# yassouali/pytorch-segmentation

Hardware: NVIDIA H100
Metric: images/sec DeepLabV3+/ResNet101 513x513 train step (fwd+CE+bwd+SGD) (higher is better)
Workload: dtype bf16

## Files before the change

### pytorch-segmentation_b200/csrc/seg_conv_tc.cu

```cuda
#include <cuda.h>
#include <mutex>
#include <stdlib.h>
#include "seg_common.cuh"
#include "seg_ptx.cuh"
#include "seg_sync.cuh"

namespace seg {
namespace tc {

using namespace ptx;

constexpr int BM = 128;
constexpr int BK = 64;
constexpr int A_BYTES = BM * 128;
constexpr int KIND_KK = 0, KIND_KM = 1;
constexpr int NTHREADS = 384;
constexpr int NCONS = 256;
constexpr int MAXT = 49;

constexpr int BAR_CONSUMERS = 1;
constexpr int BAR_ORDER = 2;
constexpr int BAR_WG = 4;

struct TcParams {
  CUtensorMap mapA;
  CUtensorMap mapB;
  int M;
  int Ncols;
  int taps;
  int kchunks;
  int stride;
  int lower_h, lower_w;
  int PQ, Q;
  int x_im2col;
  int brows_per_tap;
  short tap_wt[MAXT];
  short tap_oh[MAXT];
  short tap_ow[MAXT];
  void* out;
  long long ldo;
  int out_dtype;
  float beta;
  const float* bias;
  double* stats;
  int stat_rows;
  unsigned* stat_ticket;
  SyncDesc sync;
  int out_strided, out_H, out_W, osy, osx, opy, opx;
  int n_tiles, tiles;
  int kblocks_total, kblocks_per_split;
  float* dw;
  int dw_K, dw_C;
  float* ws;
};

__device__ __forceinline__ void row_to_coords(int m, int PQ, int Q, int stride, int lower_h, int lower_w, int& n, int& h,
                                              int& w) {
  n = m / PQ;
  int rem = m - n * PQ;
  int pp = rem / Q;
  int qq = rem - pp * Q;
  h = lower_h + pp * stride;
  w = lower_w + qq * stride;
}

template <int BN, int TA, int TB>
__device__ __forceinline__ void wgmma_tile(float* acc, uint64_t adesc, uint64_t bdesc, uint32_t accumulate) {
  if constexpr (BN == 64) wgmma_m64n64k16<TA, TB>(acc, adesc, bdesc, accumulate);
  else if constexpr (BN == 128) wgmma_m64n128k16<TA, TB>(acc, adesc, bdesc, accumulate);
  else wgmma_m64n256k16<TA, TB>(acc, adesc, bdesc, accumulate);
}

template <int BN, int KIND>
__device__ __forceinline__ void load_kblock(const TcParams& p, uint32_t a_dst, uint32_t bar, int kc, int wtap, uint16_t oh,
                                            uint16_t ow, int n_img, int h0, int w0, int m0, int n0) {
  const uint32_t b_dst = a_dst + A_BYTES;
  if (p.x_im2col)
    tma_load_im2col_4d(a_dst, &p.mapA, bar, kc * BK, w0, h0, n_img, ow, oh);
  else
    tma_load_2d(a_dst, &p.mapA, bar, kc * BK, m0);
  if (KIND == KIND_KK) {
    tma_load_2d(b_dst, &p.mapB, bar, kc * BK, wtap * p.brows_per_tap + n0);
  } else {
#pragma unroll
    for (int j = 0; j < BN / 64; ++j)
      tma_load_2d(b_dst + j * 8192, &p.mapB, bar, n0 + j * 64, wtap * p.brows_per_tap + kc * BK);
  }
}

template <int BN>
__device__ __forceinline__ void stage_acc(const float* acc, const float* acc1, uint8_t* stage, int rbase, int warp, int lane,
                                          const float* bias, bool out_f32) {
  const int esize = out_f32 ? 4 : 2;
  const int CPR = BN * esize / 16;
  const int swz = (CPR >= 32 ? 31 : CPR - 1);
  const int r0 = rbase + warp * 16 + (lane >> 2);
#pragma unroll
  for (int j = 0; j < BN / 8; ++j) {
    const int col = j * 8 + 2 * (lane & 3);
    float b0 = 0.f, b1 = 0.f;
    if (bias) {
      b0 = bias[col];
      b1 = bias[col + 1];
    }
#pragma unroll
    for (int h = 0; h < 4; ++h) {
      if (h >= 2 && !acc1) break;
      const float* a = h < 2 ? acc : acc1;
      const int r = r0 + 8 * (h & 1) + 32 * (h & 2);
      const float x0 = a[4 * j + 2 * (h & 1)] + b0, x1 = a[4 * j + 2 * (h & 1) + 1] + b1;
      const int byte = col * esize;
      uint8_t* dst = stage + (size_t)r * (BN * esize) + ((((byte >> 4) ^ (r & swz))) << 4) + (byte & 15);
      if (out_f32)
        *reinterpret_cast<float2*>(dst) = make_float2(x0, x1);
      else
        *reinterpret_cast<__nv_bfloat162*>(dst) = __floats2bfloat162_rn(x0, x1);
    }
  }
}


template <int BN, int ESIZE>
__device__ __forceinline__ void store_tile(const TcParams& p, const uint8_t* stage, int tid, int m0, int n0, int ncols_tile) {
  constexpr int CPR = BN * ESIZE / 16;
  constexpr int swz = (CPR >= 32 ? 31 : CPR - 1);
  constexpr int RSTEP = 128 / CPR;
  constexpr int NCH = BM / RSTEP;
  constexpr int BATCH = 8;
  static_assert(128 % CPR == 0 && NCH % BATCH == 0, "chunk walk of the staged tile");
  const int c16 = tid % CPR;
  const int nchunks = (ncols_tile * ESIZE + 15) >> 4;
  if (c16 >= nchunks) return;
  const bool vec_ok = ((p.ldo * ESIZE) & 15) == 0 && ((reinterpret_cast<uintptr_t>(p.out) + (size_t)n0 * ESIZE) & 15) == 0;
  const int first_col = (c16 << 4) / ESIZE;
  const bool full = first_col + 16 / ESIZE <= ncols_tile;
  auto row_dst = [&](int tr) {
    const int grow = m0 + tr;
    long long pixel = grow;
    if (p.out_strided) {
      const int n = grow / p.PQ;
      const int rem = grow - n * p.PQ;
      const int i = rem / p.Q, jj = rem - i * p.Q;
      pixel = ((long long)n * p.out_H + (i * p.osy + p.opy)) * p.out_W + (jj * p.osx + p.opx);
    }
    return reinterpret_cast<uint8_t*>(p.out) + ((size_t)pixel * p.ldo + n0) * ESIZE + ((size_t)c16 << 4);
  };
  auto row_src = [&](int tr) { return stage + (size_t)tr * (BN * ESIZE) + ((c16 ^ (tr & swz)) << 4); };
  if (ESIZE == 2 && vec_ok && full && p.beta != 0.f) {
    for (int b = 0; b < NCH; b += BATCH) {
      uint8_t* dst[BATCH];
      uint4 old[BATCH];
#pragma unroll
      for (int u = 0; u < BATCH; ++u) {
        const int tr = tid / CPR + (b + u) * RSTEP;
        dst[u] = m0 + tr < p.M ? row_dst(tr) : nullptr;
        old[u] = dst[u] ? *reinterpret_cast<const uint4*>(dst[u]) : make_uint4(0u, 0u, 0u, 0u);
      }
#pragma unroll
      for (int u = 0; u < BATCH; ++u) {
        if (!dst[u]) continue;
        float a[8], o[8];
        unpack8(*reinterpret_cast<const bf16x8*>(row_src(tid / CPR + (b + u) * RSTEP)), a);
        unpack8(*reinterpret_cast<const bf16x8*>(&old[u]), o);
#pragma unroll
        for (int k = 0; k < 8; ++k) a[k] += p.beta * o[k];
        *reinterpret_cast<bf16x8*>(dst[u]) = pack8(a);
      }
    }
    return;
  }
  for (int tr = tid / CPR; tr < BM; tr += RSTEP) {
    if (m0 + tr >= p.M) break;
    const uint8_t* src = row_src(tr);
    uint8_t* dst = row_dst(tr);
    if (ESIZE == 2 && vec_ok && full) {
      *reinterpret_cast<bf16x8*>(dst) = *reinterpret_cast<const bf16x8*>(src);
    } else if (ESIZE == 2) {
      float a[8];
      unpack8(*reinterpret_cast<const bf16x8*>(src), a);
      __nv_bfloat16* d = reinterpret_cast<__nv_bfloat16*>(dst);
      for (int k = 0; k < 8; ++k)
        if (first_col + k < ncols_tile) {
          float o = a[k];
          if (p.beta != 0.f) o += p.beta * bf2f(d[k]);
          d[k] = f2bf(o);
        }
    } else {
      const float4 val = *reinterpret_cast<const float4*>(src);
      const float a[4] = {val.x, val.y, val.z, val.w};
      float* d = reinterpret_cast<float*>(dst);
      if (vec_ok && full && p.beta == 0.f) {
        *reinterpret_cast<float4*>(d) = val;
      } else {
        for (int k = 0; k < 4; ++k)
          if (first_col + k < ncols_tile) d[k] = (p.beta != 0.f) ? a[k] + p.beta * d[k] : a[k];
      }
    }
  }
}

template <int BN>
struct PPCfg {
  static_assert(BN == 64 || BN == 128, "ping-pong tile width");
  static constexpr int B_BYTES = BN * 128;
  static constexpr int STAGE_BYTES = A_BYTES + B_BYTES;
  static constexpr int STAGES = BN == 64 ? 6 : 4;
  static constexpr int RING = STAGES * STAGE_BYTES;
  static constexpr int STG_BYTES = BM * 256;
  static constexpr int MAXG = BM / 32;
  static constexpr int STAT_BYTES = MAXG * 2 * BN * 4 + BN * 4;
  static constexpr int SMEM = RING + 2 * (STG_BYTES + STAT_BYTES) + 1024  + 256 ;
  static_assert(16 * STAGES + 8 <= 256, "barrier area");
  static_assert(SMEM <= 227 * 1024, "shared memory per block");
};

template <int BN, int KIND>
__global__ void __launch_bounds__(NTHREADS, 1) conv_gemm_pp(const __grid_constant__ TcParams p) {
  using C = PPCfg<BN>;
  constexpr int STAGES = C::STAGES;
  extern __shared__ uint8_t smem_raw[];
  const uint32_t raw_addr = smem_u32(smem_raw);
  const uint32_t smem0 = (raw_addr + 1023u) & ~1023u;
  uint8_t* smem_gen = smem_raw + (smem0 - raw_addr);
  const uint32_t bar0 = smem0 + C::RING + 2 * (C::STG_BYTES + C::STAT_BYTES);
  auto full_bar = [&](int s) { return bar0 + 8u * s; };
  auto empty_bar = [&](int s) { return bar0 + 8u * (STAGES + s); };
  volatile int* flag_sm = reinterpret_cast<volatile int*>(smem_gen + (bar0 - smem0) + 16 * STAGES);

  const int num_iters = p.taps * p.kchunks;
  const int grid = gridDim.x;
  const int ntiles = (p.tiles - (int)blockIdx.x + grid - 1) / grid;

  if (threadIdx.x == 0) {
    prefetch_tmap(&p.mapA);
    prefetch_tmap(&p.mapB);
    for (int s = 0; s < STAGES; ++s) {
      mbar_init(full_bar(s), 1);
      mbar_init(empty_bar(s), 4);
    }
    fence_mbar_init();
  }
  __syncthreads();
  pdl_wait();

  if (threadIdx.x < 128) {
    setmaxnreg_dec<40>();
    if (threadIdx.x == 0 && num_iters > 0) {
      int it = 0;
      for (int j = 0; j < ntiles; ++j) {
        const int t = blockIdx.x + j * grid;
        const int m0 = (t / p.n_tiles) * BM, n0 = (t % p.n_tiles) * BN;
        int n_img = 0, h0 = 0, w0 = 0;
        if (p.x_im2col) row_to_coords(m0, p.PQ, p.Q, p.stride, p.lower_h, p.lower_w, n_img, h0, w0);
        for (int tap = 0; tap < p.taps; ++tap) {
          const int wtap = p.tap_wt[tap];
          const uint16_t oh = (uint16_t)p.tap_oh[tap], ow = (uint16_t)p.tap_ow[tap];
          for (int kc = 0; kc < p.kchunks; ++kc, ++it) {
            const int st = it % STAGES;
            mbar_wait_nocall(empty_bar(st), ((it / STAGES) & 1) ^ 1u);
            mbar_arrive_expect_tx(full_bar(st), C::STAGE_BYTES);
            load_kblock<BN, KIND>(p, smem0 + st * C::STAGE_BYTES, full_bar(st), kc, wtap, oh, ow, n_img, h0, w0, m0, n0);
          }
        }
      }
    }
    return;
  }

  setmaxnreg_inc<232>();
  const int cw = (threadIdx.x - 128) >> 7;
  const int tid = threadIdx.x & 127;
  const int warp = tid >> 5, lane = tid & 31;
  uint8_t* stage = smem_gen + C::RING + cw * C::STG_BYTES;
  float* stat_sm = reinterpret_cast<float*>(smem_gen + C::RING + 2 * C::STG_BYTES + cw * C::STAT_BYTES);
  float* bias_sm = stat_sm + C::MAXG * 2 * BN;
  const bool out_f32 = p.out_dtype != SEG_DT_BF16;
  const int esize = out_f32 ? 4 : 2;
  const int CPR = BN * esize / 16;
  const int swz = (CPR >= 32 ? 31 : CPR - 1);
  auto wg_sync = [&] { named_sync(BAR_WG + cw, 128); };

  for (int j = cw; j < ntiles; j += 2) {
    const int t = blockIdx.x + j * grid;
    const int m0 = (t / p.n_tiles) * BM, n0 = (t % p.n_tiles) * BN;
    float acc0[BN / 2], acc1[BN / 2];
#pragma unroll
    for (int i = 0; i < BN / 2; ++i) acc0[i] = acc1[i] = 0.f;

    if (j > 0) named_sync(BAR_ORDER + cw, NCONS);
    {
      constexpr int TB = (KIND == KIND_KK) ? 0 : 1;
      const int it0 = j * num_iters;
      for (int i = 0; i < num_iters; ++i) {
        const int it = it0 + i;
        const int st = it % STAGES;
        mbar_wait_nocall(full_bar(st), (it / STAGES) & 1);
        const uint32_t a_addr = smem0 + st * C::STAGE_BYTES;
        const uint32_t b_addr = a_addr + A_BYTES;
        const uint64_t adesc0 = make_smem_desc_sw128(a_addr, 16, 1024);
        const uint64_t adesc1 = make_smem_desc_sw128(a_addr + 8192, 16, 1024);
        const uint64_t bdesc0 = make_smem_desc_sw128(b_addr, TB ? 8192 : 16, 1024);
        wgmma_fence();
#pragma unroll
        for (int k = 0; k < BK / 16; ++k) {
          const uint64_t bdesc = bdesc0 + (uint64_t)(TB ? (k * 2048 >> 4) : (k * 32 >> 4));
          wgmma_tile<BN, 0, TB>(acc0, adesc0 + (uint64_t)(k * 32 >> 4), bdesc, 1u);
          wgmma_tile<BN, 0, TB>(acc1, adesc1 + (uint64_t)(k * 32 >> 4), bdesc, 1u);
        }
        wgmma_commit();
        wgmma_wait<1>();
        __syncwarp();
        if (i > 0 && lane == 0) mbar_arrive(empty_bar((it - 1) % STAGES));
      }
      if (j + 1 < ntiles) named_arrive(BAR_ORDER + (cw ^ 1), NCONS);
      wgmma_wait<0>();
      __syncwarp();
      if (num_iters > 0 && lane == 0) mbar_arrive(empty_bar((it0 + num_iters - 1) % STAGES));
    }

    const int ncols_tile = min(BN, p.Ncols - n0);
    if (p.bias && tid < BN) bias_sm[tid] = tid < ncols_tile ? __ldg(p.bias + n0 + tid) : 0.f;
    wg_sync();
    stage_acc<BN>(acc0, acc1, stage, 0, warp, lane, p.bias ? bias_sm : nullptr, out_f32);
    wg_sync();

    const int ngroups = BM / p.stat_rows;
    if (p.stats) {
      const int parts = min(128 / BN, ngroups);
      const int rpp = BM / parts;
      const int c = tid % BN, part = tid / BN;
      const int rvalid = min(BM, p.M - m0);
      if (part < parts) {
        const int byte = c * esize;
        int g = part * rpp / p.stat_rows;
        auto load = [&](int r) {
          const uint8_t* src = stage + (size_t)r * (BN * esize) + ((((byte >> 4) ^ (r & swz))) << 4) + (byte & 15);
          return out_f32 ? *reinterpret_cast<const float*>(src) : bf2f(*reinterpret_cast<const __nv_bfloat16*>(src));
        };
        for (int rg = part * rpp; rg < (part + 1) * rpp; rg += p.stat_rows, ++g) {
          float s1 = 0.f, s2 = 0.f;
          const int rend = min(rg + p.stat_rows, rvalid);
          int r = rg;
          for (; r + 8 <= rend; r += 8) {
            float x[8];
#pragma unroll
            for (int u = 0; u < 8; ++u) x[u] = load(r + u);
#pragma unroll
            for (int u = 0; u < 8; ++u) {
              s1 += x[u];
              s2 = fmaf(x[u], x[u], s2);
            }
          }
          for (; r < rend; ++r) {
            const float x = load(r);
            s1 += x;
            s2 = fmaf(x, x, s2);
          }
          stat_sm[(g * 2 + 0) * BN + c] = s1;
          stat_sm[(g * 2 + 1) * BN + c] = s2;
        }
      }
    }

    if (out_f32)
      store_tile<BN, 4>(p, stage, tid, m0, n0, ncols_tile);
    else
      store_tile<BN, 2>(p, stage, tid, m0, n0, ncols_tile);
    if (j == ntiles - 1 && tid == 0) pdl_trigger();

    if (p.stats) {
      wg_sync();
      if (tid < ncols_tile) {
        float a = 0.f, b = 0.f;
        for (int g = 0; g < ngroups; ++g) {
          a += stat_sm[(g * 2 + 0) * BN + tid];
          b += stat_sm[(g * 2 + 1) * BN + tid];
        }
        atomicAdd(p.stats + n0 + tid, (double)a);
        atomicAdd(p.stats + p.Ncols + n0 + tid, (double)b);
      }
    }
  }

  if (p.stats && p.sync.world > 0)
    sync_push_when_last<false>(p.sync, p.stats, 2 * p.Ncols, p.stat_ticket, gridDim.x, threadIdx.x - 128, NCONS,
                               [] { named_sync(BAR_CONSUMERS, NCONS); }, flag_sm);
}


template <int BN>
struct Cfg {
  static constexpr int B_BYTES = BN * 128;
  static constexpr int STAGE_BYTES = A_BYTES + B_BYTES;
  static constexpr int STAGES = BN == 64 ? 6 : (BN == 128 ? 5 : 4);
  static constexpr int SMEM = STAGES * STAGE_BYTES + 1024  + 256 ;
  static_assert(STAGES * STAGE_BYTES >= BM * BN * 4, "staging tile must fit in the pipeline ring");
  static_assert(SMEM <= 227 * 1024, "shared memory per block");
};

template <int BN>
__global__ void __launch_bounds__(NTHREADS, 1) conv_gemm_wgrad(const __grid_constant__ TcParams p) {
  using C = Cfg<BN>;
  constexpr int STAGES = C::STAGES;
  extern __shared__ uint8_t smem_raw[];
  const uint32_t raw_addr = smem_u32(smem_raw);
  const uint32_t smem0 = (raw_addr + 1023u) & ~1023u;
  uint8_t* smem_gen = smem_raw + (smem0 - raw_addr);
  const uint32_t bar0 = smem0 + STAGES * C::STAGE_BYTES;
  auto full_bar = [&](int s) { return bar0 + 8u * s; };
  auto empty_bar = [&](int s) { return bar0 + 8u * (STAGES + s); };

  const int m0 = blockIdx.x * BM;
  const int n0 = blockIdx.y * BN;

  const int tap_mm = blockIdx.z % p.taps;
  const int split = blockIdx.z / p.taps;
  const int kb_begin = split * p.kblocks_per_split;
  const int kb_end = min(kb_begin + p.kblocks_per_split, p.kblocks_total);
  const int num_iters = max(kb_end - kb_begin, 0);

  if (threadIdx.x == 0) {
    prefetch_tmap(&p.mapA);
    prefetch_tmap(&p.mapB);
    for (int s = 0; s < STAGES; ++s) {
      mbar_init(full_bar(s), 1);
      mbar_init(empty_bar(s), 8);
    }
    fence_mbar_init();
  }
  __syncthreads();
  pdl_wait();

  if (threadIdx.x < 128) {
    if (threadIdx.x == 0 && num_iters > 0) {
      const uint16_t oh = (uint16_t)p.tap_oh[tap_mm], ow = (uint16_t)p.tap_ow[tap_mm];
      int it = 0;
      for (int kb = kb_begin; kb < kb_end; ++kb, ++it) {
        const int st = it % STAGES;
        const uint32_t ph = (it / STAGES) & 1;
        mbar_wait_nocall(empty_bar(st), ph ^ 1u);
        const uint32_t a_dst = smem0 + st * C::STAGE_BYTES;
        const uint32_t b_dst = a_dst + A_BYTES;
        const int pix0 = kb * BK;
        mbar_arrive_expect_tx(full_bar(st), C::STAGE_BYTES);
        tma_load_2d(a_dst, &p.mapA, full_bar(st), m0, pix0);
        tma_load_2d(a_dst + 8192, &p.mapA, full_bar(st), m0 + 64, pix0);
        if (p.x_im2col) {
          int n_img, h0, w0;
          row_to_coords(pix0, p.PQ, p.Q, p.stride, p.lower_h, p.lower_w, n_img, h0, w0);
#pragma unroll
          for (int j = 0; j < BN / 64; ++j)
            tma_load_im2col_4d(b_dst + j * 8192, &p.mapB, full_bar(st), n0 + j * 64, w0, h0, n_img, ow, oh);
        } else {
#pragma unroll
          for (int j = 0; j < BN / 64; ++j) tma_load_2d(b_dst + j * 8192, &p.mapB, full_bar(st), n0 + j * 64, pix0);
        }
      }
    }
    return;
  }

  if (num_iters == 0) return;
  const int ctid = threadIdx.x - 128;
  const int cw = ctid >> 7;
  const int warp = (ctid >> 5) & 3, lane = ctid & 31;
  float acc[BN / 2];
#pragma unroll
  for (int i = 0; i < BN / 2; ++i) acc[i] = 0.f;
  for (int it = 0; it < num_iters; ++it) {
    const int st = it % STAGES;
    mbar_wait_nocall(full_bar(st), (it / STAGES) & 1);
    const uint32_t a_addr = smem0 + st * C::STAGE_BYTES + cw * 8192;
    const uint32_t b_addr = smem0 + st * C::STAGE_BYTES + A_BYTES;
    const uint64_t adesc0 = make_smem_desc_sw128(a_addr, 8192, 1024);
    const uint64_t bdesc0 = make_smem_desc_sw128(b_addr, 8192, 1024);
    wgmma_fence();
#pragma unroll
    for (int k = 0; k < BK / 16; ++k)
      wgmma_tile<BN, 1, 1>(acc, adesc0 + (uint64_t)(k * 2048 >> 4), bdesc0 + (uint64_t)(k * 2048 >> 4), 1u);
    wgmma_commit();
    wgmma_wait<1>();
    __syncwarp();
    if (it > 0 && lane == 0) mbar_arrive(empty_bar((it - 1) % STAGES));
  }
  wgmma_wait<0>();
  named_sync(BAR_CONSUMERS, NCONS);

  uint8_t* stage = smem_gen;
  const int ncols_tile = min(BN, p.Ncols - n0);
  stage_acc<BN>(acc, nullptr, stage, cw * 64, warp, lane, nullptr, true);
  named_sync(BAR_CONSUMERS, NCONS);

  const int CPR = BN * 4 / 16;
  const int swz = (CPR >= 32 ? 31 : CPR - 1);
  float* base = p.ws ? p.ws + (size_t)split * p.taps * p.dw_K * p.dw_C : p.dw;
  for (int idx = ctid; idx < BM * CPR; idx += NCONS) {
    const int tr = idx / CPR, c16 = idx - tr * CPR;
    const int row = m0 + tr, col0 = c16 * 4;
    if (row >= p.M || col0 >= ncols_tile) continue;
    const float4 v = *reinterpret_cast<const float4*>(stage + (size_t)tr * (BN * 4) + ((c16 ^ (tr & swz)) << 4));
    float* dst = base + ((size_t)tap_mm * p.dw_K + row) * p.dw_C + n0 + col0;
    const bool vec = col0 + 4 <= ncols_tile && ((reinterpret_cast<uintptr_t>(dst) & 15) == 0);
    const float a[4] = {v.x, v.y, v.z, v.w};
    if (p.ws) {
      if (vec)
        *reinterpret_cast<float4*>(dst) = v;
      else
        for (int i = 0; i < 4; ++i)
          if (col0 + i < ncols_tile) dst[i] = a[i];
    } else if (vec) {
      asm volatile("red.global.add.v4.f32 [%0], {%1, %2, %3, %4};" ::"l"(dst), "f"(v.x), "f"(v.y), "f"(v.z), "f"(v.w)
                   : "memory");
    } else {
      for (int i = 0; i < 4; ++i)
        if (col0 + i < ncols_tile) atomicAdd(dst + i, a[i]);
    }
  }
}

typedef CUresult (*EncodeTiledFn)(CUtensorMap*, CUtensorMapDataType, cuuint32_t, void*, const cuuint64_t*,
                                  const cuuint64_t*, const cuuint32_t*, const cuuint32_t*, CUtensorMapInterleave,
                                  CUtensorMapSwizzle, CUtensorMapL2promotion, CUtensorMapFloatOOBfill);
typedef CUresult (*EncodeIm2colFn)(CUtensorMap*, CUtensorMapDataType, cuuint32_t, void*, const cuuint64_t*,
                                   const cuuint64_t*, const int*, const int*, cuuint32_t, cuuint32_t,
                                   const cuuint32_t*, CUtensorMapInterleave, CUtensorMapSwizzle,
                                   CUtensorMapL2promotion, CUtensorMapFloatOOBfill);
static EncodeTiledFn g_encode_tiled = nullptr;
static EncodeIm2colFn g_encode_im2col = nullptr;
static int g_driver_version = 0;

static int resolve_driver() {
  static std::once_flag once;
  static int status = 0;
  std::call_once(once, [] {
    void* f1 = nullptr;
    void* f2 = nullptr;
    cudaDriverEntryPointQueryResult q;
    if (cudaGetDriverEntryPoint("cuTensorMapEncodeTiled", &f1, cudaEnableDefault, &q) != cudaSuccess || !f1) status = 1;
    if (cudaGetDriverEntryPoint("cuTensorMapEncodeIm2col", &f2, cudaEnableDefault, &q) != cudaSuccess || !f2) status = 1;
    g_encode_tiled = (EncodeTiledFn)f1;
    g_encode_im2col = (EncodeIm2colFn)f2;
    cudaDriverGetVersion(&g_driver_version);
  });
  if (status) set_error("cannot resolve cuTensorMapEncode* driver entry points");
  return status;
}

static int make_map_2d(CUtensorMap* m, const void* ptr, int64_t rows, int64_t cols, int64_t ld, int box_rows) {
  if (resolve_driver()) return 1;
  SEG_REQUIRE((reinterpret_cast<uintptr_t>(ptr) & 15) == 0, "TMA: base pointer not 16-byte aligned");
  SEG_REQUIRE(ld % 8 == 0, "TMA: row pitch %lld not a multiple of 8 elements", (long long)ld);
  cuuint64_t dims[2] = {(cuuint64_t)cols, (cuuint64_t)rows};
  cuuint64_t strides[1] = {(cuuint64_t)ld * 2};
  cuuint32_t box[2] = {64, (cuuint32_t)box_rows};
  cuuint32_t es[2] = {1, 1};
  CUresult r = g_encode_tiled(m, CU_TENSOR_MAP_DATA_TYPE_BFLOAT16, 2, const_cast<void*>(ptr), dims, strides, box, es,
                              CU_TENSOR_MAP_INTERLEAVE_NONE, CU_TENSOR_MAP_SWIZZLE_128B,
                              CU_TENSOR_MAP_L2_PROMOTION_L2_256B, CU_TENSOR_MAP_FLOAT_OOB_FILL_NONE);
  SEG_REQUIRE(r == CUDA_SUCCESS, "cuTensorMapEncodeTiled failed (%d) rows=%lld cols=%lld ld=%lld box_rows=%d", (int)r,
              (long long)rows, (long long)cols, (long long)ld, box_rows);
  return 0;
}

static int make_map_im2col(CUtensorMap* m, const void* ptr, int N, int H, int W, int C, int64_t ld, int lower_w,
                           int lower_h, int upper_w, int upper_h, int stride, int pixels) {
  if (resolve_driver()) return 1;
  SEG_REQUIRE((reinterpret_cast<uintptr_t>(ptr) & 15) == 0, "TMA: base pointer not 16-byte aligned");
  SEG_REQUIRE(ld % 8 == 0, "TMA: channel pitch %lld not a multiple of 8", (long long)ld);
  SEG_REQUIRE(lower_w >= -128 && upper_w >= -128 && lower_w <= 127 && upper_w <= 127 && lower_h >= -128 &&
                  upper_h >= -128 && lower_h <= 127 && upper_h <= 127,
              "im2col corner out of range");
  cuuint64_t dims[4] = {(cuuint64_t)C, (cuuint64_t)W, (cuuint64_t)H, (cuuint64_t)N};
  cuuint64_t strides[3] = {(cuuint64_t)ld * 2, (cuuint64_t)W * ld * 2, (cuuint64_t)H * W * ld * 2};
  int lo[2] = {lower_w, lower_h};
  int up[2] = {upper_w, upper_h};
  cuuint32_t es[4] = {1, (cuuint32_t)stride, (cuuint32_t)stride, 1};
  CUresult r = g_encode_im2col(m, CU_TENSOR_MAP_DATA_TYPE_BFLOAT16, 4, const_cast<void*>(ptr), dims, strides, lo, up,
                               64, (cuuint32_t)pixels, es, CU_TENSOR_MAP_INTERLEAVE_NONE, CU_TENSOR_MAP_SWIZZLE_128B,
                               CU_TENSOR_MAP_L2_PROMOTION_L2_256B, CU_TENSOR_MAP_FLOAT_OOB_FILL_NONE);
  SEG_REQUIRE(r == CUDA_SUCCESS,
              "cuTensorMapEncodeIm2col failed (%d) N=%d H=%d W=%d C=%d ld=%lld lo=(%d,%d) up=(%d,%d) s=%d", (int)r, N, H,
              W, C, (long long)ld, lower_w, lower_h, upper_w, upper_h, stride);
  if (g_driver_version <= 13010) {
    const uint64_t bytes = (uint64_t)N * H * W * ld * 2;
    if (bytes < 131072) reinterpret_cast<uint64_t*>(m)[1] &= ~(1ull << 21);
  }
  return 0;
}

template <int BN, int KIND>
static int launch_pp(TcParams& p, cudaStream_t stream) {
  static bool attr_set = false;
  auto kfn = conv_gemm_pp<BN, KIND>;
  if (!attr_set) {
    cudaError_t e = cudaFuncSetAttribute(kfn, cudaFuncAttributeMaxDynamicSharedMemorySize, PPCfg<BN>::SMEM);
    SEG_REQUIRE(e == cudaSuccess, "cudaFuncSetAttribute(smem=%d): %s", PPCfg<BN>::SMEM, cudaGetErrorString(e));
    attr_set = true;
  }
  const int n_tiles = ceil_div(p.Ncols, BN);
  const int64_t tiles = ceil_div64(p.M, BM) * n_tiles;
  SEG_REQUIRE(tiles < (1ll << 31), "too many output tiles");
  p.n_tiles = n_tiles;
  p.tiles = (int)tiles;
  const dim3 grid((unsigned)std::min<int64_t>(tiles, num_sms()));
  launch_pdl(kfn, grid, dim3(NTHREADS), (size_t)PPCfg<BN>::SMEM, stream, p);
  return check_launch("conv_gemm_pp");
}

template <int KIND>
static int launch_pp_bn(int bn, TcParams& p, cudaStream_t stream) {
  switch (bn) {
    case 64: return launch_pp<64, KIND>(p, stream);
    case 128: return launch_pp<128, KIND>(p, stream);
  }
  set_error("bad BN %d", bn);
  return 1;
}

template <int BN>
static int launch_wgrad(const TcParams& p, dim3 grid, cudaStream_t stream) {
  static bool attr_set = false;
  auto kfn = conv_gemm_wgrad<BN>;
  if (!attr_set) {
    cudaError_t e = cudaFuncSetAttribute(kfn, cudaFuncAttributeMaxDynamicSharedMemorySize, Cfg<BN>::SMEM);
    SEG_REQUIRE(e == cudaSuccess, "cudaFuncSetAttribute(smem=%d): %s", Cfg<BN>::SMEM, cudaGetErrorString(e));
    attr_set = true;
  }
  launch_pdl(kfn, grid, dim3(NTHREADS), (size_t)Cfg<BN>::SMEM, stream, p);
  return check_launch("conv_gemm_wgrad");
}

static int launch_wgrad_bn(int bn, const TcParams& p, dim3 grid, cudaStream_t stream) {
  switch (bn) {
    case 64: return launch_wgrad<64>(p, grid, stream);
    case 128: return launch_wgrad<128>(p, grid, stream);
    case 256: return launch_wgrad<256>(p, grid, stream);
  }
  set_error("bad BN %d", bn);
  return 1;
}

static int pick_bn(int ncols, bool out_f32) { return (ncols <= 64 || out_f32) ? 64 : 128; }

static int stat_rows_for(int ncols) {
  if (ncols <= 64) return 32;
  if (ncols < 256) return 64;
  return ceil_div(ncols, 256) * 256 - ncols < 128 ? 128 : 64;
}

bool supported(const seg_conv_desc* d) {
  if (d->C % 8 != 0 || d->ldx % 8 != 0) return false;
  if (d->R != d->S) return false;
  if (d->R * d->S > MAXT) return false;
  if (d->pad > 127 || d->dil * (d->R - 1) - d->pad > 127 || d->dil * (d->R - 1) - d->pad < -127) return false;
  if (d->stride > 8) return false;
  return true;
}

static bool is_pointwise(const seg_conv_desc* d) { return d->R == 1 && d->S == 1 && d->stride == 1 && d->pad == 0; }

int conv_fwd(const seg_conv_desc* d, const void* x, const void* w, void* y, int y_dtype, const float* bias, float beta,
             double* stats, unsigned* stat_ticket, const SyncDesc* sync, cudaStream_t stream) {
  SEG_REQUIRE(supported(d), "wgmma conv fwd: unsupported shape (C=%d ldx=%d R=%d pad=%d dil=%d)", d->C, d->ldx, d->R,
              d->pad, d->dil);
  TcParams p;
  memset(&p, 0, sizeof(p));
  const int64_t M = (int64_t)d->N * d->P * d->Q;
  SEG_REQUIRE(M < (1ll << 31), "M too large");
  p.M = (int)M;
  p.Ncols = d->K;
  p.taps = d->R * d->S;
  for (int t = 0; t < p.taps; ++t) {
    p.tap_wt[t] = (short)t;
    p.tap_oh[t] = (short)((t / d->S) * d->dil);
    p.tap_ow[t] = (short)((t % d->S) * d->dil);
  }
  p.kchunks = ceil_div(d->C, BK);
  p.stride = d->stride;
  p.lower_h = p.lower_w = -d->pad;
  p.PQ = d->P * d->Q;
  p.Q = d->Q;
  p.brows_per_tap = d->K;
  p.out = y;
  p.ldo = d->ldy;
  p.out_dtype = y_dtype;
  p.beta = beta;
  p.bias = bias;
  p.stats = stats;
  p.stat_ticket = stat_ticket;
  if (sync && stats) {
    SEG_REQUIRE(stat_ticket != nullptr, "conv fwd: SyncBN needs a zeroed ticket word");
    SEG_REQUIRE(4 * d->K <= sync->n_max, "conv fwd: 2*K = %d fp64 statistics exceed the SyncBN buffer (%d floats)", 2 * d->K, sync->n_max);
    p.sync = *sync;
  }
  const int bn = pick_bn(d->K, y_dtype != SEG_DT_BF16);
  p.stat_rows = stat_rows_for(d->K);
  if (is_pointwise(d)) {
    p.x_im2col = 0;
    if (make_map_2d(&p.mapA, x, M, d->C, d->ldx, BM)) return 1;
  } else {
    p.x_im2col = 1;
    const int upper = d->pad - (d->R - 1) * d->dil;
    if (make_map_im2col(&p.mapA, x, d->N, d->H, d->W, d->C, d->ldx, -d->pad, -d->pad, upper, upper, d->stride, BM)) return 1;
  }
  if (make_map_2d(&p.mapB, w, (int64_t)p.taps * d->K, d->C, d->C, bn)) return 1;
  return launch_pp_bn<KIND_KK>(bn, p, stream);
}

static int floordiv(int a, int b) { return (a >= 0) ? a / b : -((-a + b - 1) / b); }

int conv_dgrad(const seg_conv_desc* d, const void* dy, const void* w, void* dx, float beta, cudaStream_t stream) {
  SEG_REQUIRE(supported(d) && d->ldy % 8 == 0, "wgmma conv dgrad: unsupported shape (stride=%d K=%d ldy=%d)", d->stride,
              d->K, d->ldy);
  const int s = d->stride;
  const int bn = pick_bn(d->C, false);
  for (int py = 0; py < s; ++py) {
    for (int px = 0; px < s; ++px) {
      const int Hs = (d->H - py + s - 1) / s, Ws = (d->W - px + s - 1) / s;
      if (Hs <= 0 || Ws <= 0) continue;
      TcParams p;
      memset(&p, 0, sizeof(p));
      int rh[8], oh[8], nh = 0, rw[8], ow[8], nw = 0;
      for (int r = 0; r < d->R; ++r) {
        const int num = py + d->pad - r * d->dil;
        if (((num % s) + s) % s == 0) { rh[nh] = r; oh[nh] = floordiv(num, s); ++nh; }
      }
      for (int q = 0; q < d->S; ++q) {
        const int num = px + d->pad - q * d->dil;
        if (((num % s) + s) % s == 0) { rw[nw] = q; ow[nw] = floordiv(num, s); ++nw; }
      }
      int min_oh = 0, min_ow = 0;
      for (int i = 0; i < nh; ++i) min_oh = (i == 0) ? oh[i] : min(min_oh, oh[i]);
      for (int i = 0; i < nw; ++i) min_ow = (i == 0) ? ow[i] : min(min_ow, ow[i]);
      p.taps = nh * nw;
      for (int i = 0; i < nh; ++i)
        for (int j = 0; j < nw; ++j) {
          const int t = i * nw + j;
          p.tap_wt[t] = (short)(rh[i] * d->S + rw[j]);
          p.tap_oh[t] = (short)(oh[i] - min_oh);
          p.tap_ow[t] = (short)(ow[j] - min_ow);
        }
      const int64_t M = (int64_t)d->N * Hs * Ws;
      SEG_REQUIRE(M < (1ll << 31), "M too large");
      p.M = (int)M;
      p.Ncols = d->C;
      p.kchunks = ceil_div(d->K, BK);
      p.stride = 1;
      p.lower_h = min_oh;
      p.lower_w = min_ow;
      p.PQ = Hs * Ws;
      p.Q = Ws;
      p.brows_per_tap = d->K;
      p.out = dx;
      p.ldo = d->ldx;
      p.out_dtype = SEG_DT_BF16;
      p.beta = beta;
      if (s > 1) {
        p.out_strided = 1;
        p.out_H = d->H;
        p.out_W = d->W;
        p.osy = p.osx = s;
        p.opy = py;
        p.opx = px;
      }
      p.stat_rows = BM;
      if (p.taps > 0) {
        const bool plain = (s == 1 && is_pointwise(d));
        if (plain) {
          p.x_im2col = 0;
          if (make_map_2d(&p.mapA, dy, M, d->K, d->ldy, BM)) return 1;
        } else {
          p.x_im2col = 1;
          const int upper_h = Hs - d->P + min_oh, upper_w = Ws - d->Q + min_ow;
          if (make_map_im2col(&p.mapA, dy, d->N, d->P, d->Q, d->K, d->ldy, min_ow, min_oh, upper_w, upper_h, 1, BM)) return 1;
        }
        if (make_map_2d(&p.mapB, w, (int64_t)d->R * d->S * d->K, d->C, d->C, 64)) return 1;
      } else {
        if (beta == 1.f) continue;
        if (make_map_2d(&p.mapA, w, (int64_t)d->R * d->S * d->K, d->C, d->C, BM)) return 1;
        if (make_map_2d(&p.mapB, w, (int64_t)d->R * d->S * d->K, d->C, d->C, 64)) return 1;
      }
      if (launch_pp_bn<KIND_KM>(bn, p, stream)) return 1;
    }
  }
  return 0;
}

__global__ void wgrad_split_reduce_kernel(const float* __restrict__ ws, int splits, int64_t n, float* __restrict__ dw) {
  for (int64_t i = blockIdx.x * (int64_t)blockDim.x + threadIdx.x; i < n; i += (int64_t)gridDim.x * blockDim.x) {
    float acc = ws[i];
    for (int s = 1; s < splits; ++s) acc += ws[(size_t)s * n + i];
    dw[i] += acc;
  }
}

static void wgrad_plan(const seg_conv_desc* d, int& bn, int& splits, int& kblocks_per_split) {
  const bool wide = d->R * d->S >= 9 && d->C >= 256 && d->C % 256 == 0;
  bn = (d->C <= 64) ? 64 : (wide ? 256 : 128);
  const int kblocks_total = (int)ceil_div64((int64_t)d->N * d->P * d->Q, BK);
  const int tiles = ceil_div(d->K, BM) * ceil_div(d->C, bn) * d->R * d->S;
  splits = max(1, num_sms() / tiles);
  splits = min(splits, kblocks_total);
  splits = min(splits, 1024);
  kblocks_per_split = ceil_div(kblocks_total, splits);
  splits = ceil_div(kblocks_total, kblocks_per_split);
}

int64_t wgrad_workspace_floats(const seg_conv_desc* d) {
  if (!supported(d)) return 0;
  int bn, splits, kps;
  wgrad_plan(d, bn, splits, kps);
  return splits > 1 ? (int64_t)splits * d->R * d->S * d->K * d->C : 0;
}

int conv_wgrad(const seg_conv_desc* d, const void* dy, const void* x, float* dw, float* ws, cudaStream_t stream) {
  SEG_REQUIRE(supported(d) && d->ldy % 8 == 0, "wgmma conv wgrad: unsupported shape");
  TcParams p;
  memset(&p, 0, sizeof(p));
  const int64_t npix = (int64_t)d->N * d->P * d->Q;
  SEG_REQUIRE(npix < (1ll << 31), "too many pixels");
  p.M = d->K;
  p.Ncols = d->C;
  p.taps = d->R * d->S;
  for (int t = 0; t < p.taps; ++t) {
    p.tap_wt[t] = (short)t;
    p.tap_oh[t] = (short)((t / d->S) * d->dil);
    p.tap_ow[t] = (short)((t % d->S) * d->dil);
  }
  p.stride = d->stride;
  p.lower_h = p.lower_w = -d->pad;
  p.PQ = d->P * d->Q;
  p.Q = d->Q;
  p.dw = dw;
  p.dw_K = d->K;
  p.dw_C = d->C;
  p.kblocks_total = (int)ceil_div64(npix, BK);
  int bn, splits;
  wgrad_plan(d, bn, splits, p.kblocks_per_split);
  SEG_REQUIRE(splits == 1 || ws != nullptr, "wgmma conv wgrad: %d k-splits need the workspace (seg_conv2d_wgrad_workspace_floats)", splits);
  SEG_REQUIRE((int64_t)(splits - 1) * p.kblocks_per_split < p.kblocks_total, "wgmma conv wgrad: split %d has no k-blocks", splits - 1);
  if (splits > 1) p.ws = ws;
  if (make_map_2d(&p.mapA, dy, npix, d->K, d->ldy, 64)) return 1;
  if (is_pointwise(d)) {
    p.x_im2col = 0;
    if (make_map_2d(&p.mapB, x, npix, d->C, d->ldx, 64)) return 1;
  } else {
    p.x_im2col = 1;
    const int upper = d->pad - (d->R - 1) * d->dil;
    if (make_map_im2col(&p.mapB, x, d->N, d->H, d->W, d->C, d->ldx, -d->pad, -d->pad, upper, upper, d->stride, 64)) return 1;
  }
  SEG_REQUIRE((unsigned)(p.taps * splits) <= 65535u, "wgrad grid.z too large");
  dim3 grid((unsigned)ceil_div(d->K, BM), (unsigned)ceil_div(d->C, bn), (unsigned)(p.taps * splits));
  if (launch_wgrad_bn(bn, p, grid, stream)) return 1;
  if (splits == 1) return 0;
  const int64_t n = (int64_t)p.taps * d->K * d->C;
  wgrad_split_reduce_kernel<<<(unsigned)std::min<int64_t>(ceil_div64(n, 256), (int64_t)num_sms() * 8), 256, 0, stream>>>(ws, splits, n, dw);
  return check_launch("wgrad_split_reduce");
}

}
}
```

Measured before the change: 372.9.

## Make wgrad GEMM persistent with direct register epilogue and register rebalancing

Converts the weight-gradient conv GEMM from one CTA per tile into a persistent kernel. Each CTA walks (split, tap, m, n) units in a grid-stride loop while the TMA producer keeps the smem ring full across tile boundaries. The epilogue no longer stages accumulators through shared memory with extra barriers: each thread writes or reduces its fragments directly to global as float2 stores or red.add. Producer and consumer warpgroups also rebalance registers with setmaxnreg. The aim is to hide prologue and epilogue latency and cut launch and tail waste, at the cost of less-coalesced global writes from the fragment layout.

```diff
diff --git a/pytorch-segmentation_b200/csrc/seg_conv_tc.cu b/pytorch-segmentation_b200/csrc/seg_conv_tc.cu
--- a/pytorch-segmentation_b200/csrc/seg_conv_tc.cu
+++ b/pytorch-segmentation_b200/csrc/seg_conv_tc.cu
@@ -394,9 +394,20 @@
   static constexpr int STAGE_BYTES = A_BYTES + B_BYTES;
   static constexpr int STAGES = BN == 64 ? 6 : (BN == 128 ? 5 : 4);
   static constexpr int SMEM = STAGES * STAGE_BYTES + 1024  + 256 ;
-  static_assert(STAGES * STAGE_BYTES >= BM * BN * 4, "staging tile must fit in the pipeline ring");
+  static_assert(16 * STAGES <= 256, "barrier area");
   static_assert(SMEM <= 227 * 1024, "shared memory per block");
 };
+
+template <int BN>
+__device__ __forceinline__ void wgrad_unit(const TcParams& p, int u, int& split, int& tap, int& m0, int& n0) {
+  split = u / p.tiles;
+  int t = u - split * p.tiles;
+  const int mtiles = (p.M + BM - 1) / BM;
+  m0 = (t % mtiles) * BM;
+  t /= mtiles;
+  n0 = (t % p.n_tiles) * BN;
+  tap = t / p.n_tiles;
+}
 
 template <int BN>
 __global__ void __launch_bounds__(NTHREADS, 1) conv_gemm_wgrad(const __grid_constant__ TcParams p) {
@@ -405,19 +416,13 @@
   extern __shared__ uint8_t smem_raw[];
   const uint32_t raw_addr = smem_u32(smem_raw);
   const uint32_t smem0 = (raw_addr + 1023u) & ~1023u;
-  uint8_t* smem_gen = smem_raw + (smem0 - raw_addr);
   const uint32_t bar0 = smem0 + STAGES * C::STAGE_BYTES;
   auto full_bar = [&](int s) { return bar0 + 8u * s; };
   auto empty_bar = [&](int s) { return bar0 + 8u * (STAGES + s); };
 
-  const int m0 = blockIdx.x * BM;
-  const int n0 = blockIdx.y * BN;
-
-  const int tap_mm = blockIdx.z % p.taps;
-  const int split = blockIdx.z / p.taps;
-  const int kb_begin = split * p.kblocks_per_split;
-  const int kb_end = min(kb_begin + p.kblocks_per_split, p.kblocks_total);
-  const int num_iters = max(kb_end - kb_begin, 0);
+  const int splits = (p.kblocks_total + p.kblocks_per_split - 1) / p.kblocks_per_split;
+  const int grid = gridDim.x;
+  const int nunits = (p.tiles * splits - (int)blockIdx.x + grid - 1) / grid;
 
   if (threadIdx.x == 0) {
     prefetch_tmap(&p.mapA);
@@ -432,88 +437,103 @@
   pdl_wait();
 
   if (threadIdx.x < 128) {
-    if (threadIdx.x == 0 && num_iters > 0) {
-      const uint16_t oh = (uint16_t)p.tap_oh[tap_mm], ow = (uint16_t)p.tap_ow[tap_mm];
+    setmaxnreg_dec<40>();
+    if (threadIdx.x == 0) {
       int it = 0;
-      for (int kb = kb_begin; kb < kb_end; ++kb, ++it) {
-        const int st = it % STAGES;
-        const uint32_t ph = (it / STAGES) & 1;
-        mbar_wait_nocall(empty_bar(st), ph ^ 1u);
-        const uint32_t a_dst = smem0 + st * C::STAGE_BYTES;
-        const uint32_t b_dst = a_dst + A_BYTES;
-        const int pix0 = kb * BK;
-        mbar_arrive_expect_tx(full_bar(st), C::STAGE_BYTES);
-        tma_load_2d(a_dst, &p.mapA, full_bar(st), m0, pix0);
-        tma_load_2d(a_dst + 8192, &p.mapA, full_bar(st), m0 + 64, pix0);
-        if (p.x_im2col) {
-          int n_img, h0, w0;
-          row_to_coords(pix0, p.PQ, p.Q, p.stride, p.lower_h, p.lower_w, n_img, h0, w0);
-#pragma unroll
-          for (int j = 0; j < BN / 64; ++j)
-            tma_load_im2col_4d(b_dst + j * 8192, &p.mapB, full_bar(st), n0 + j * 64, w0, h0, n_img, ow, oh);
-        } else {
-#pragma unroll
-          for (int j = 0; j < BN / 64; ++j) tma_load_2d(b_dst + j * 8192, &p.mapB, full_bar(st), n0 + j * 64, pix0);
+      for (int j = 0; j < nunits; ++j) {
+        int split, tap, m0, n0;
+        wgrad_unit<BN>(p, blockIdx.x + j * grid, split, tap, m0, n0);
+        const uint16_t oh = (uint16_t)p.tap_oh[tap], ow = (uint16_t)p.tap_ow[tap];
+        const int kb_begin = split * p.kblocks_per_split;
+        const int kb_end = min(kb_begin + p.kblocks_per_split, p.kblocks_total);
+        for (int kb = kb_begin; kb < kb_end; ++kb, ++it) {
+          const int st = it % STAGES;
+          mbar_wait_nocall(empty_bar(st), ((it / STAGES) & 1) ^ 1u);
+          const uint32_t a_dst = smem0 + st * C::STAGE_BYTES;
+          const uint32_t b_dst = a_dst + A_BYTES;
+          const int pix0 = kb * BK;
+          mbar_arrive_expect_tx(full_bar(st), C::STAGE_BYTES);
+          tma_load_2d(a_dst, &p.mapA, full_bar(st), m0, pix0);
+          tma_load_2d(a_dst + 8192, &p.mapA, full_bar(st), m0 + 64, pix0);
+          if (p.x_im2col) {
+            int n_img, h0, w0;
+            row_to_coords(pix0, p.PQ, p.Q, p.stride, p.lower_h, p.lower_w, n_img, h0, w0);
+#pragma unroll
+            for (int c = 0; c < BN / 64; ++c)
+              tma_load_im2col_4d(b_dst + c * 8192, &p.mapB, full_bar(st), n0 + c * 64, w0, h0, n_img, ow, oh);
+          } else {
+#pragma unroll
+            for (int c = 0; c < BN / 64; ++c) tma_load_2d(b_dst + c * 8192, &p.mapB, full_bar(st), n0 + c * 64, pix0);
+          }
         }
       }
     }
     return;
   }
 
-  if (num_iters == 0) return;
+  setmaxnreg_inc<232>();
   const int ctid = threadIdx.x - 128;
   const int cw = ctid >> 7;
   const int warp = (ctid >> 5) & 3, lane = ctid & 31;
-  float acc[BN / 2];
-#pragma unroll
-  for (int i = 0; i < BN / 2; ++i) acc[i] = 0.f;
-  for (int it = 0; it < num_iters; ++it) {
-    const int st = it % STAGES;
-    mbar_wait_nocall(full_bar(st), (it / STAGES) & 1);
-    const uint32_t a_addr = smem0 + st * C::STAGE_BYTES + cw * 8192;
-    const uint32_t b_addr = smem0 + st * C::STAGE_BYTES + A_BYTES;
-    const uint64_t adesc0 = make_smem_desc_sw128(a_addr, 8192, 1024);
-    const uint64_t bdesc0 = make_smem_desc_sw128(b_addr, 8192, 1024);
-    wgmma_fence();
-#pragma unroll
-    for (int k = 0; k < BK / 16; ++k)
-      wgmma_tile<BN, 1, 1>(acc, adesc0 + (uint64_t)(k * 2048 >> 4), bdesc0 + (uint64_t)(k * 2048 >> 4), 1u);
-    wgmma_commit();
-    wgmma_wait<1>();
+  int it = 0;
+  for (int j = 0; j < nunits; ++j) {
+    int split, tap, m0, n0;
+    wgrad_unit<BN>(p, blockIdx.x + j * grid, split, tap, m0, n0);
+    const int kb_begin = split * p.kblocks_per_split;
+    const int num_iters = min(kb_begin + p.kblocks_per_split, p.kblocks_total) - kb_begin;
+    float acc[BN / 2];
+#pragma unroll
+    for (int i = 0; i < BN / 2; ++i) acc[i] = 0.f;
+    for (int i = 0; i < num_iters; ++i, ++it) {
+      const int st = it % STAGES;
+      mbar_wait_nocall(full_bar(st), (it / STAGES) & 1);
+      const uint32_t a_addr = smem0 + st * C::STAGE_BYTES + cw * 8192;
+      const uint32_t b_addr = smem0 + st * C::STAGE_BYTES + A_BYTES;
+      const uint64_t adesc0 = make_smem_desc_sw128(a_addr, 8192, 1024);
+      const uint64_t bdesc0 = make_smem_desc_sw128(b_addr, 8192, 1024);
+      wgmma_fence();
+#pragma unroll
+      for (int k = 0; k < BK / 16; ++k)
+        wgmma_tile<BN, 1, 1>(acc, adesc0 + (uint64_t)(k * 2048 >> 4), bdesc0 + (uint64_t)(k * 2048 >> 4), 1u);
+      wgmma_commit();
+      wgmma_wait<1>();
+      __syncwarp();
+      if (i > 0 && lane == 0) mbar_arrive(empty_bar((it - 1) % STAGES));
+    }
+    wgmma_wait<0>();
     __syncwarp();
-    if (it > 0 && lane == 0) mbar_arrive(empty_bar((it - 1) % STAGES));
-  }
-  wgmma_wait<0>();
-  named_sync(BAR_CONSUMERS, NCONS);
-
-  uint8_t* stage = smem_gen;
-  const int ncols_tile = min(BN, p.Ncols - n0);
-  stage_acc<BN>(acc, nullptr, stage, cw * 64, warp, lane, nullptr, true);
-  named_sync(BAR_CONSUMERS, NCONS);
-
-  const int CPR = BN * 4 / 16;
-  const int swz = (CPR >= 32 ? 31 : CPR - 1);
-  float* base = p.ws ? p.ws + (size_t)split * p.taps * p.dw_K * p.dw_C : p.dw;
-  for (int idx = ctid; idx < BM * CPR; idx += NCONS) {
-    const int tr = idx / CPR, c16 = idx - tr * CPR;
-    const int row = m0 + tr, col0 = c16 * 4;
-    if (row >= p.M || col0 >= ncols_tile) continue;
-    const float4 v = *reinterpret_cast<const float4*>(stage + (size_t)tr * (BN * 4) + ((c16 ^ (tr & swz)) << 4));
-    float* dst = base + ((size_t)tap_mm * p.dw_K + row) * p.dw_C + n0 + col0;
-    const bool vec = col0 + 4 <= ncols_tile && ((reinterpret_cast<uintptr_t>(dst) & 15) == 0);
-    const float a[4] = {v.x, v.y, v.z, v.w};
-    if (p.ws) {
-      if (vec)
-        *reinterpret_cast<float4*>(dst) = v;
-      else
-        for (int i = 0; i < 4; ++i)
-          if (col0 + i < ncols_tile) dst[i] = a[i];
-    } else if (vec) {
-      asm volatile("red.global.add.v4.f32 [%0], {%1, %2, %3, %4};" ::"l"(dst), "f"(v.x), "f"(v.y), "f"(v.z), "f"(v.w)
-                   : "memory");
-    } else {
-      for (int i = 0; i < 4; ++i)
-        if (col0 + i < ncols_tile) atomicAdd(dst + i, a[i]);
+    if (lane == 0) mbar_arrive(empty_bar((it - 1) % STAGES));
+
+    const int ncols_tile = min(BN, p.Ncols - n0);
+    float* base = p.ws ? p.ws + (size_t)split * p.taps * p.dw_K * p.dw_C : p.dw;
+    const int r0 = m0 + cw * 64 + warp * 16 + (lane >> 2);
+#pragma unroll
+    for (int h = 0; h < 2; ++h) {
+      const int row = r0 + 8 * h;
+      if (row >= p.M) continue;
+      float* drow = base + ((size_t)tap * p.dw_K + row) * p.dw_C + n0;
+      const bool vec = (reinterpret_cast<uintptr_t>(drow) & 7) == 0;
+#pragma unroll
+      for (int c8 = 0; c8 < BN / 8; ++c8) {
+        const int col = c8 * 8 + 2 * (lane & 3);
+        if (col >= ncols_tile) continue;
+        const float v0 = acc[4 * c8 + 2 * h], v1 = acc[4 * c8 + 2 * h + 1];
+        float* dst = drow + col;
+        if (vec && col + 2 <= ncols_tile) {
+          if (p.ws)
+            *reinterpret_cast<float2*>(dst) = make_float2(v0, v1);
+          else
+            asm volatile("red.global.add.v2.f32 [%0], {%1, %2};" ::"l"(dst), "f"(v0), "f"(v1) : "memory");
+        } else {
+          if (p.ws) {
+            dst[0] = v0;
+            if (col + 1 < ncols_tile) dst[1] = v1;
+          } else {
+            atomicAdd(dst, v0);
+            if (col + 1 < ncols_tile) atomicAdd(dst + 1, v1);
+          }
+        }
+      }
     }
   }
 }
@@ -618,7 +638,7 @@
 }
 
 template <int BN>
-static int launch_wgrad(const TcParams& p, dim3 grid, cudaStream_t stream) {
+static int launch_wgrad(const TcParams& p, int units, cudaStream_t stream) {
   static bool attr_set = false;
   auto kfn = conv_gemm_wgrad<BN>;
   if (!attr_set) {
@@ -626,15 +646,15 @@
     SEG_REQUIRE(e == cudaSuccess, "cudaFuncSetAttribute(smem=%d): %s", Cfg<BN>::SMEM, cudaGetErrorString(e));
     attr_set = true;
   }
-  launch_pdl(kfn, grid, dim3(NTHREADS), (size_t)Cfg<BN>::SMEM, stream, p);
+  launch_pdl(kfn, dim3((unsigned)std::min(units, num_sms())), dim3(NTHREADS), (size_t)Cfg<BN>::SMEM, stream, p);
   return check_launch("conv_gemm_wgrad");
 }
 
-static int launch_wgrad_bn(int bn, const TcParams& p, dim3 grid, cudaStream_t stream) {
+static int launch_wgrad_bn(int bn, const TcParams& p, int units, cudaStream_t stream) {
   switch (bn) {
-    case 64: return launch_wgrad<64>(p, grid, stream);
-    case 128: return launch_wgrad<128>(p, grid, stream);
-    case 256: return launch_wgrad<256>(p, grid, stream);
+    case 64: return launch_wgrad<64>(p, units, stream);
+    case 128: return launch_wgrad<128>(p, units, stream);
+    case 256: return launch_wgrad<256>(p, units, stream);
   }
   set_error("bad BN %d", bn);
   return 1;
@@ -849,9 +869,11 @@
     const int upper = d->pad - (d->R - 1) * d->dil;
     if (make_map_im2col(&p.mapB, x, d->N, d->H, d->W, d->C, d->ldx, -d->pad, -d->pad, upper, upper, d->stride, 64)) return 1;
   }
-  SEG_REQUIRE((unsigned)(p.taps * splits) <= 65535u, "wgrad grid.z too large");
-  dim3 grid((unsigned)ceil_div(d->K, BM), (unsigned)ceil_div(d->C, bn), (unsigned)(p.taps * splits));
-  if (launch_wgrad_bn(bn, p, grid, stream)) return 1;
+  p.n_tiles = ceil_div(d->C, bn);
+  const int64_t tiles = ceil_div64(d->K, BM) * p.n_tiles * p.taps;
+  SEG_REQUIRE(tiles * splits < (1ll << 31), "too many wgrad units");
+  p.tiles = (int)tiles;
+  if (launch_wgrad_bn(bn, p, (int)(tiles * splits), stream)) return 1;
   if (splits == 1) return 0;
   const int64_t n = (int64_t)p.taps * d->K * d->C;
   wgrad_split_reduce_kernel<<<(unsigned)std::min<int64_t>(ceil_div64(n, 256), (int64_t)num_sms() * 8), 256, 0, stream>>>(ws, splits, n, dw);
```

After: 374.9 (median of 6 runs). About the same (+0.5%).
